# ZhengyiLuo/PHC

Measured on NVIDIA H100. Metric: env-steps/sec (fused obs+reward+PPO) at 4096 envs/GPU, higher is better.
Workload: dtype f32

## Files before the change

phc_b200/csrc/gemm_wgmma.cu:

```cuda
#include <cuda_runtime.h>
#include <stdint.h>
#include <stdlib.h>
#include <string.h>

#include "../../include/phc_b200.h"
#include "phc_common.cuh"

extern "C" void phc_set_error(const char* msg);
extern "C" int phc_check_cuda(cudaError_t e, const char* what);
extern "C" void phc_count_launches(int n);

namespace phc {
namespace wg {

constexpr int BM = 128, NUM_THREADS = 256, MAX_PROBLEMS = PHC_GEMM_GROUP_MAX;

template <int BN>
struct Cfg {
  static constexpr int BK = BN == 128 ? 32 : 16;
  static constexpr int A_TILE = BM * BK * 4;
  static constexpr int B_TILE = BN * BK * 4;
  static constexpr int STAGE = 2 * (A_TILE + B_TILE);
  static constexpr int SMEM = 2 * STAGE;
  static constexpr int SBO = BK * 32;
  static constexpr int A_PER = BM * BK / NUM_THREADS;
  static constexpr int B_PER = BN * BK / NUM_THREADS;
};

struct Prob {
  const float* A; const float* B; const float* A_lo; const float* B_lo;
  float* C; float* C_hi; float* C_lo;
  const float* bias;
  float* aux;
  long long lda, ldb, ldc, ldaux;
  int M, N, K;
  float alpha;
  int act, accumulate, a_k, b_k, k_splits;
  int tiles_m, tiles_n, kb_total, kb_per, tile_begin, tile_count;
  unsigned int* turn;
  int turn_first, turn_total;
};

struct Params {
  Prob p[MAX_PROBLEMS];
  int count, total_tiles;
  unsigned int* sched;
  int single_pass;
};

__device__ __forceinline__ void wgmma_tf32_n128(float (&d)[64], uint64_t da, uint64_t db) {
  asm volatile(
      "{\n\t.reg .pred p;\n\tsetp.ne.b32 p, 1, 0;\n\t"
      "wgmma.mma_async.sync.aligned.m64n128k8.f32.tf32.tf32 {%0, %1, %2, %3, %4, %5, %6, %7, %8, %9, %10, %11, %12, %13, %14, %15, %16, %17, %18, %19, %20, %21, %22, %23, %24, %25, %26, %27, %28, %29, %30, %31, %32, %33, %34, %35, %36, %37, %38, %39, %40, %41, %42, %43, %44, %45, %46, %47, %48, %49, %50, %51, %52, %53, %54, %55, %56, %57, %58, %59, %60, %61, %62, %63}, %64, %65, p, 1, 1;\n\t}"
      : "+f"(d[0]), "+f"(d[1]), "+f"(d[2]), "+f"(d[3]), "+f"(d[4]), "+f"(d[5]), "+f"(d[6]), "+f"(d[7]), "+f"(d[8]), "+f"(d[9]), "+f"(d[10]), "+f"(d[11]), "+f"(d[12]), "+f"(d[13]), "+f"(d[14]), "+f"(d[15]), "+f"(d[16]), "+f"(d[17]), "+f"(d[18]), "+f"(d[19]), "+f"(d[20]), "+f"(d[21]), "+f"(d[22]), "+f"(d[23]), "+f"(d[24]), "+f"(d[25]), "+f"(d[26]), "+f"(d[27]), "+f"(d[28]), "+f"(d[29]), "+f"(d[30]), "+f"(d[31]), "+f"(d[32]), "+f"(d[33]), "+f"(d[34]), "+f"(d[35]), "+f"(d[36]), "+f"(d[37]), "+f"(d[38]), "+f"(d[39]), "+f"(d[40]), "+f"(d[41]), "+f"(d[42]), "+f"(d[43]), "+f"(d[44]), "+f"(d[45]), "+f"(d[46]), "+f"(d[47]), "+f"(d[48]), "+f"(d[49]), "+f"(d[50]), "+f"(d[51]), "+f"(d[52]), "+f"(d[53]), "+f"(d[54]), "+f"(d[55]), "+f"(d[56]), "+f"(d[57]), "+f"(d[58]), "+f"(d[59]), "+f"(d[60]), "+f"(d[61]), "+f"(d[62]), "+f"(d[63])
      : "l"(da), "l"(db));
}
__device__ __forceinline__ void wgmma_tf32_n256(float (&d)[128], uint64_t da, uint64_t db) {
  asm volatile(
      "{\n\t.reg .pred p;\n\tsetp.ne.b32 p, 1, 0;\n\t"
      "wgmma.mma_async.sync.aligned.m64n256k8.f32.tf32.tf32 {%0, %1, %2, %3, %4, %5, %6, %7, %8, %9, %10, %11, %12, %13, %14, %15, %16, %17, %18, %19, %20, %21, %22, %23, %24, %25, %26, %27, %28, %29, %30, %31, %32, %33, %34, %35, %36, %37, %38, %39, %40, %41, %42, %43, %44, %45, %46, %47, %48, %49, %50, %51, %52, %53, %54, %55, %56, %57, %58, %59, %60, %61, %62, %63, %64, %65, %66, %67, %68, %69, %70, %71, %72, %73, %74, %75, %76, %77, %78, %79, %80, %81, %82, %83, %84, %85, %86, %87, %88, %89, %90, %91, %92, %93, %94, %95, %96, %97, %98, %99, %100, %101, %102, %103, %104, %105, %106, %107, %108, %109, %110, %111, %112, %113, %114, %115, %116, %117, %118, %119, %120, %121, %122, %123, %124, %125, %126, %127}, %128, %129, p, 1, 1;\n\t}"
      : "+f"(d[0]), "+f"(d[1]), "+f"(d[2]), "+f"(d[3]), "+f"(d[4]), "+f"(d[5]), "+f"(d[6]), "+f"(d[7]), "+f"(d[8]), "+f"(d[9]), "+f"(d[10]), "+f"(d[11]), "+f"(d[12]), "+f"(d[13]), "+f"(d[14]), "+f"(d[15]), "+f"(d[16]), "+f"(d[17]), "+f"(d[18]), "+f"(d[19]), "+f"(d[20]), "+f"(d[21]), "+f"(d[22]), "+f"(d[23]), "+f"(d[24]), "+f"(d[25]), "+f"(d[26]), "+f"(d[27]), "+f"(d[28]), "+f"(d[29]), "+f"(d[30]), "+f"(d[31]), "+f"(d[32]), "+f"(d[33]), "+f"(d[34]), "+f"(d[35]), "+f"(d[36]), "+f"(d[37]), "+f"(d[38]), "+f"(d[39]), "+f"(d[40]), "+f"(d[41]), "+f"(d[42]), "+f"(d[43]), "+f"(d[44]), "+f"(d[45]), "+f"(d[46]), "+f"(d[47]), "+f"(d[48]), "+f"(d[49]), "+f"(d[50]), "+f"(d[51]), "+f"(d[52]), "+f"(d[53]), "+f"(d[54]), "+f"(d[55]), "+f"(d[56]), "+f"(d[57]), "+f"(d[58]), "+f"(d[59]), "+f"(d[60]), "+f"(d[61]), "+f"(d[62]), "+f"(d[63]), "+f"(d[64]), "+f"(d[65]), "+f"(d[66]), "+f"(d[67]), "+f"(d[68]), "+f"(d[69]), "+f"(d[70]), "+f"(d[71]), "+f"(d[72]), "+f"(d[73]), "+f"(d[74]), "+f"(d[75]), "+f"(d[76]), "+f"(d[77]), "+f"(d[78]), "+f"(d[79]), "+f"(d[80]), "+f"(d[81]), "+f"(d[82]), "+f"(d[83]), "+f"(d[84]), "+f"(d[85]), "+f"(d[86]), "+f"(d[87]), "+f"(d[88]), "+f"(d[89]), "+f"(d[90]), "+f"(d[91]), "+f"(d[92]), "+f"(d[93]), "+f"(d[94]), "+f"(d[95]), "+f"(d[96]), "+f"(d[97]), "+f"(d[98]), "+f"(d[99]), "+f"(d[100]), "+f"(d[101]), "+f"(d[102]), "+f"(d[103]), "+f"(d[104]), "+f"(d[105]), "+f"(d[106]), "+f"(d[107]), "+f"(d[108]), "+f"(d[109]), "+f"(d[110]), "+f"(d[111]), "+f"(d[112]), "+f"(d[113]), "+f"(d[114]), "+f"(d[115]), "+f"(d[116]), "+f"(d[117]), "+f"(d[118]), "+f"(d[119]), "+f"(d[120]), "+f"(d[121]), "+f"(d[122]), "+f"(d[123]), "+f"(d[124]), "+f"(d[125]), "+f"(d[126]), "+f"(d[127])
      : "l"(da), "l"(db));
}

__device__ __forceinline__ void wgmma_fence() { asm volatile("wgmma.fence.sync.aligned;" ::: "memory"); }
__device__ __forceinline__ void wgmma_commit() { asm volatile("wgmma.commit_group.sync.aligned;" ::: "memory"); }
__device__ __forceinline__ void wgmma_wait_all() { asm volatile("wgmma.wait_group.sync.aligned 0;" ::: "memory"); }

__device__ __forceinline__ uint64_t smem_desc(uint32_t addr, uint32_t lbo, uint32_t sbo) {
  return (uint64_t)((addr & 0x3FFFF) >> 4) | ((uint64_t)(lbo >> 4) << 16) | ((uint64_t)(sbo >> 4) << 32);
}

template <int BN, typename Acc>
__device__ __forceinline__ void wgmma_tf32(Acc& d, uint64_t da, uint64_t db) {
  if constexpr (BN == 128) wgmma_tf32_n128(d, da, db); else wgmma_tf32_n256(d, da, db);
}

__device__ __forceinline__ float trunc_hi(float x) { return __uint_as_float(__float_as_uint(x) & 0xFFFFE000u); }
__device__ __forceinline__ float split_lo(float x) {
  const float d = x - trunc_hi(x);
  return __uint_as_float((__float_as_uint(d) + 0x1000u) & 0xFFFFE000u);
}
__device__ __forceinline__ void sts128(uint32_t addr, float a, float b, float c, float d) {
  asm volatile("st.shared.v4.f32 [%0], {%1, %2, %3, %4};" ::"r"(addr), "f"(a), "f"(b), "f"(c), "f"(d) : "memory");
}
__device__ __forceinline__ void sts32(uint32_t addr, float a) { asm volatile("st.shared.f32 [%0], %1;" ::"r"(addr), "f"(a) : "memory"); }

template <int R, int BK>
struct Map {
  static constexpr int KC = BK / 4;
  __device__ static void kmaj(int c, int& r, int& kc) { r = (c & 7) + 8 * (c / (8 * KC)); kc = (c >> 3) % KC; }
  __device__ static void mnmaj(int e, int& r, int& k, uint32_t& off) {
    const int rl = e & 7, kl = (e >> 3) & 3, e2 = e >> 5, rh = e2 % (R / 8), kh = e2 / (R / 8);
    r = rh * 8 + rl; k = kh * 4 + kl;
    off = (uint32_t)(rh * BK * 32 + kh * 128 + rl * 16 + kl * 4);
  }
};

template <int R, int BK, int PER>
__device__ __forceinline__ void load_op(float (&v)[PER], const float* __restrict__ g, long long ld, bool kmaj, int r0, int rows, int k0,
                                        int K, int tid) {
  using Mp = Map<R, BK>;
  if (kmaj) {
#pragma unroll
    for (int i = 0; i < PER / 4; ++i) {
      int r, kc;
      Mp::kmaj(tid + i * NUM_THREADS, r, kc);
      const int rr = r0 + r, kk = k0 + 4 * kc;
      const float* src = g + (long long)rr * ld + kk;
      if (rr < rows && kk + 3 < K) {
        const float4 t = *reinterpret_cast<const float4*>(src);
        v[4 * i] = t.x; v[4 * i + 1] = t.y; v[4 * i + 2] = t.z; v[4 * i + 3] = t.w;
      } else {
#pragma unroll
        for (int e = 0; e < 4; ++e) v[4 * i + e] = (rr < rows && kk + e < K) ? src[e] : 0.f;
      }
    }
  } else {
#pragma unroll
    for (int i = 0; i < PER; ++i) {
      int r, k;
      uint32_t off;
      Mp::mnmaj(tid + i * NUM_THREADS, r, k, off);
      const int rr = r0 + r, kk = k0 + k;
      v[i] = (rr < rows && kk < K) ? g[(long long)kk * ld + rr] : 0.f;
    }
  }
}

template <int R, int BK, int PER, int MODE>
__device__ __forceinline__ void store_op(const float (&v)[PER], const float (&w)[PER], uint32_t s_hi, uint32_t s_lo, bool kmaj, int tid) {
  using Mp = Map<R, BK>;
  auto hi = [](float x) { return MODE == 2 ? x : trunc_hi(x); };
  if (kmaj) {
#pragma unroll
    for (int i = 0; i < PER / 4; ++i) {
      const uint32_t off = (uint32_t)(tid + i * NUM_THREADS) * 16u;
      sts128(s_hi + off, hi(v[4 * i]), hi(v[4 * i + 1]), hi(v[4 * i + 2]), hi(v[4 * i + 3]));
      if (MODE == 0) sts128(s_lo + off, split_lo(v[4 * i]), split_lo(v[4 * i + 1]), split_lo(v[4 * i + 2]), split_lo(v[4 * i + 3]));
      if (MODE == 2) sts128(s_lo + off, w[4 * i], w[4 * i + 1], w[4 * i + 2], w[4 * i + 3]);
    }
  } else {
#pragma unroll
    for (int i = 0; i < PER; ++i) {
      int r, k;
      uint32_t off;
      Mp::mnmaj(tid + i * NUM_THREADS, r, k, off);
      sts32(s_hi + off, hi(v[i]));
      if (MODE == 0) sts32(s_lo + off, split_lo(v[i]));
      if (MODE == 2) sts32(s_lo + off, w[i]);
    }
  }
}

__device__ __forceinline__ void split_rna(float x, float& h, float& l) {
  uint32_t a, b;
  asm("cvt.rna.tf32.f32 %0, %1;" : "=r"(a) : "f"(x));
  const float res = x - __uint_as_float(a);
  asm("cvt.rna.tf32.f32 %0, %1;" : "=r"(b) : "f"(res));
  h = __uint_as_float(a); l = __uint_as_float(b);
}

template <int BN, bool PRESPLIT>
__global__ void __launch_bounds__(NUM_THREADS, 1) gemm_wgmma_kernel(const __grid_constant__ Params P) {
  using C = Cfg<BN>;
  constexpr int BK = C::BK;
  extern __shared__ __align__(128) uint8_t smem[];
  __shared__ int s_tile;
  const int tid = threadIdx.x, lane = tid & 31, wgi = tid >> 7, wq = (tid >> 5) & 3;
  const uint32_t sbase = (uint32_t)__cvta_generic_to_shared(smem);
  const bool dyn = P.sched != nullptr;
  const bool single = !PRESPLIT && P.single_pass != 0;

  for (int it = 0;; ++it) {
    int t;
    if (dyn) {
      if (tid == 0) s_tile = (int)atomicAdd(P.sched, 1u);
      __syncthreads();
      t = s_tile;
      __syncthreads();
    } else {
      t = blockIdx.x + it * gridDim.x;
    }
    if (t >= P.total_tiles) break;
    int gi = 0;
#pragma unroll 1
    while (gi + 1 < P.count && t >= P.p[gi].tile_begin + P.p[gi].tile_count) ++gi;
    const Prob& q = P.p[gi];
    const int tl = t - q.tile_begin;
    const int ni = tl % q.tiles_n, rr = tl / q.tiles_n, mi = rr % q.tiles_m, z = rr / q.tiles_m;
    const int m0 = mi * BM, n0 = ni * BN;
    const int kb_begin = z * q.kb_per;
    const int nkb = max(0, min(q.kb_total, kb_begin + q.kb_per) - kb_begin);
    if (nkb == 0) continue;
    const bool ak = q.a_k != 0, bk = q.b_k != 0;

    float acc[BN / 2];
#pragma unroll
    for (int j = 0; j < BN / 2; ++j) acc[j] = 0.f;
    float va[C::A_PER], vb[C::B_PER], wa[PRESPLIT ? C::A_PER : 1], wb[PRESPLIT ? C::B_PER : 1];
    constexpr int MODE = PRESPLIT ? 2 : 0;
    auto load = [&](int kb) {
      const int k0 = kb * BK;
      load_op<BM, BK>(va, q.A, q.lda, ak, m0, q.M, k0, q.K, tid);
      load_op<BN, BK>(vb, q.B, q.ldb, bk, n0, q.N, k0, q.K, tid);
      if constexpr (PRESPLIT) {
        load_op<BM, BK>(wa, q.A_lo, q.lda, ak, m0, q.M, k0, q.K, tid);
        load_op<BN, BK>(wb, q.B_lo, q.ldb, bk, n0, q.N, k0, q.K, tid);
      }
    };
    auto store = [&](int buf) {
      const uint32_t s = sbase + (uint32_t)(buf * C::STAGE);
      if (single) {
        store_op<BM, BK, C::A_PER, 1>(va, va, s, 0, ak, tid);
        store_op<BN, BK, C::B_PER, 1>(vb, vb, s + 2 * C::A_TILE, 0, bk, tid);
      } else if constexpr (PRESPLIT) {
        store_op<BM, BK, C::A_PER, 2>(va, wa, s, s + C::A_TILE, ak, tid);
        store_op<BN, BK, C::B_PER, 2>(vb, wb, s + 2 * C::A_TILE, s + 2 * C::A_TILE + C::B_TILE, bk, tid);
      } else {
        store_op<BM, BK, C::A_PER, MODE>(va, va, s, s + C::A_TILE, ak, tid);
        store_op<BN, BK, C::B_PER, MODE>(vb, vb, s + 2 * C::A_TILE, s + 2 * C::A_TILE + C::B_TILE, bk, tid);
      }
      fence_async_smem();
    };

    load(kb_begin);
    store(0);
    __syncthreads();
#pragma unroll 1
    for (int i = 0; i < nkb; ++i) {
      const uint32_t s = sbase + (uint32_t)((i & 1) * C::STAGE);
      const uint32_t a_hi = s + (uint32_t)(wgi * 8 * C::SBO), a_lo = a_hi + C::A_TILE;
      const uint32_t b_hi = s + 2 * C::A_TILE, b_lo = b_hi + C::B_TILE;
      wgmma_fence();
#pragma unroll
      for (int kk = 0; kk < BK / 8; ++kk) {
        const uint32_t o = (uint32_t)kk * 256u;
        const uint64_t dAh = smem_desc(a_hi + o, 128, C::SBO), dBh = smem_desc(b_hi + o, 128, C::SBO);
        if (!single) {
          wgmma_tf32<BN>(acc, smem_desc(a_lo + o, 128, C::SBO), dBh);
          wgmma_tf32<BN>(acc, dAh, smem_desc(b_lo + o, 128, C::SBO));
        }
        wgmma_tf32<BN>(acc, dAh, dBh);
      }
      wgmma_commit();
      if (i + 1 < nkb) {
        load(kb_begin + i + 1);
        store((i + 1) & 1);
      }
      wgmma_wait_all();
      __syncthreads();
    }

    const bool ordered = q.turn != nullptr;
    volatile unsigned int* turn = ordered ? q.turn + mi * q.tiles_n + ni : nullptr;
    if (ordered) {
      if (tid == 0) {
        while (*turn != (unsigned)(q.turn_first + z)) __nanosleep(64);
        __threadfence();
      }
      __syncthreads();
    }
    const int act = q.act;
    const float* bias = (q.bias && z == 0) ? q.bias : nullptr;
#pragma unroll
    for (int h = 0; h < 2; ++h) {
      const int m = m0 + wgi * 64 + wq * 16 + (lane >> 2) + 8 * h;
      const bool row_ok = m < q.M;
      float* crow = q.C + (long long)m * q.ldc;
      float* arow = (q.aux && act < PHC_ACT_RELU_BITS && row_ok) ? q.aux + (long long)m * q.ldaux : nullptr;
      uint32_t* brow = (q.aux && act >= PHC_ACT_RELU_BITS && row_ok) ? reinterpret_cast<uint32_t*>(q.aux) + (long long)m * q.ldaux : nullptr;
#pragma unroll
      for (int qc = 0; qc < BN / 32; ++qc) {
        const int nb = n0 + 32 * qc;
        if (nb >= q.N) break;
        const uint32_t mbits = (act == PHC_ACT_MASK_BITS && brow) ? brow[nb >> 5] : 0u;
        uint32_t bits = 0;
#pragma unroll
        for (int jj = 0; jj < 4; ++jj) {
          const int j = 4 * qc + jj;
          const int nl = 8 * jj + 2 * (lane & 3);
          float v[2];
#pragma unroll
          for (int c = 0; c < 2; ++c) {
            const int n = nb + nl + c;
            float x = q.alpha * acc[4 * j + 2 * h + c];
            if (bias && n < q.N) x += bias[n];
            if (act == PHC_ACT_RELU || act == PHC_ACT_RELU_BITS) x = fmaxf(x, 0.f);
            if (act == PHC_ACT_RELU_BITS) bits |= (x > 0.f ? 1u : 0u) << (nl + c);
            else if (act == PHC_ACT_MASK_BITS) x = ((mbits >> (nl + c)) & 1u) ? x : 0.f;
            else if (arow && n < q.N) {
              if (act == PHC_ACT_SILU) { arow[n] = x; x = silu_f(x); }
              else if (act == PHC_ACT_SILU_BWD) x *= silu_grad_f(arow[n]);
              else x = arow[n] > 0.f ? x : 0.f;
// ... 1 lines not shown
              x = silu_f(x);
            }
            v[c] = x;
          }
          if (!row_ok) continue;
          const int n = nb + nl;
          if (ordered) {
            if (n < q.N) crow[n] = __ldcg(crow + n) + v[0];
            if (n + 1 < q.N) crow[n + 1] = __ldcg(crow + n + 1) + v[1];
          } else if (q.accumulate) {
            if (n < q.N) atomicAdd(crow + n, v[0]);
            if (n + 1 < q.N) atomicAdd(crow + n + 1, v[1]);
          } else if (n + 1 < q.N) {
            *reinterpret_cast<float2*>(crow + n) = make_float2(v[0], v[1]);
          } else if (n < q.N) {
            crow[n] = v[0];
          }
          if (PRESPLIT && q.C_hi) {
            float h0, l0, h1, l1;
            split_rna(v[0], h0, l0); split_rna(v[1], h1, l1);
            if (n < q.N) { q.C_hi[(long long)m * q.ldc + n] = h0; q.C_lo[(long long)m * q.ldc + n] = l0; }
            if (n + 1 < q.N) { q.C_hi[(long long)m * q.ldc + n + 1] = h1; q.C_lo[(long long)m * q.ldc + n + 1] = l1; }
          }
        }
        if (act == PHC_ACT_RELU_BITS) {
          bits |= __shfl_xor_sync(0xffffffffu, bits, 1);
          bits |= __shfl_xor_sync(0xffffffffu, bits, 2);
          if (brow && (lane & 3) == 0) brow[nb >> 5] = bits;
        }
      }
    }
    if (ordered) {
      __threadfence();
      __syncthreads();
      if (tid == 0) *turn = (q.turn_first + z + 1 == q.turn_total) ? 0u : (unsigned)(q.turn_first + z + 1);
    }
  }
  if (dyn && tid == 0 && atomicInc(P.sched + 1, gridDim.x - 1) == gridDim.x - 1) { __threadfence(); P.sched[0] = 0u; }
}

__global__ void split_lo_kernel(const float* __restrict__ x, float* __restrict__ lo, int64_t n) {
  const int64_t stride = (int64_t)gridDim.x * blockDim.x;
  for (int64_t i = (int64_t)blockIdx.x * blockDim.x + threadIdx.x; i < n; i += stride) lo[i] = split_lo(x[i]);
}

__global__ void split_tf32_kernel(const float* __restrict__ x, int64_t ldx, int64_t rows, int cols, float* __restrict__ hi,
                                  float* __restrict__ lo, int64_t ldo) {
  const int64_t total = rows * cols;
  for (int64_t i = (int64_t)blockIdx.x * blockDim.x + threadIdx.x; i < total; i += (int64_t)gridDim.x * blockDim.x) {
    const int64_t r = i / cols;
    const int c = (int)(i - r * cols);
    split_rna(x[r * ldx + c], hi[r * ldo + c], lo[r * ldo + c]);
  }
}

static int g_single_pass = 0;
static int g_tile = 0;
static int g_sched = -1;
constexpr int SCHED_SLOTS = 64;
__device__ unsigned int g_sched_counters[SCHED_SLOTS][2];
constexpr int TURN_SLOTS = 16, TURN_TILES = 8192;
__device__ unsigned int g_turns[TURN_SLOTS][TURN_TILES];

static int num_sms() {
  static int n = 0;
  if (!n) { int dev = 0; cudaGetDevice(&dev); cudaDeviceGetAttribute(&n, cudaDevAttrMultiProcessorCount, dev); if (n <= 0) n = 132; }
  return n;
}

static int add_problem(Params& P, int n, int tiles, int bn, const float* A, const float* A_lo, long long lda, int a_k, const float* B,
                       const float* B_lo, long long ldb, int b_k, float* Cm, float* C_hi, float* C_lo, long long ldc, int M, int N, int K,
                       float alpha, const float* bias, int act, float* aux, long long ldaux, int accumulate, int k_splits) {
  const int bk = bn == 128 ? Cfg<128>::BK : Cfg<256>::BK;
  Prob& q = P.p[n];
  q.A = A; q.A_lo = A_lo; q.B = B; q.B_lo = B_lo; q.C = Cm; q.C_hi = C_hi; q.C_lo = C_lo; q.bias = bias; q.aux = aux;
  q.lda = lda; q.ldb = ldb; q.ldc = ldc; q.ldaux = ldaux; q.M = M; q.N = N; q.K = K; q.alpha = alpha; q.act = act;
  q.accumulate = accumulate ? 1 : 0; q.a_k = a_k ? 1 : 0; q.b_k = b_k ? 1 : 0;
  int ks = k_splits < 1 ? 1 : k_splits;
  q.tiles_m = (M + BM - 1) / BM;
  q.tiles_n = (N + bn - 1) / bn;
  q.kb_total = (K + bk - 1) / bk;
  if (ks > q.kb_total) ks = q.kb_total;
  q.kb_per = (q.kb_total + ks - 1) / ks;
  ks = (q.kb_total + q.kb_per - 1) / q.kb_per;
  q.k_splits = ks;
  q.turn = nullptr;
  q.tile_begin = tiles;
  q.tile_count = q.tiles_m * q.tiles_n * ks;
  return q.tile_count;
}

template <int BN, bool PRESPLIT>
static int launch(Params& P, bool dynamic_sched, cudaStream_t stream) {
  int owner[MAX_PROBLEMS];
  bool ordered = false;
  int turn_tiles = 0;
  for (int i = 0; i < P.count; ++i) {
    Prob& q = P.p[i];
    owner[i] = -1;
    for (int j = 0; j < i && q.accumulate; ++j) {
// ... 20 lines not shown
      void* p = nullptr;
      cudaError_t es = cudaGetSymbolAddress(&p, g_turns);
      if (es != cudaSuccess) return phc_check_cuda(es, "cudaGetSymbolAddress(g_turns)");
      tbase = static_cast<unsigned int*>(p);
    }
    unsigned int* t = tbase + (size_t)(turn_no++ % TURN_SLOTS) * TURN_TILES;
    for (int i = 0; i < P.count; ++i) {
      Prob& q = P.p[i];
      if (owner[i] >= 0) {
        Prob& o = P.p[owner[i]];
        q.turn = o.turn;
        q.turn_first = o.turn_total;
        o.turn_total += q.k_splits;
      } else if (q.k_splits > 1 || has_members[i]) {
        q.turn = t; t += q.tiles_m * q.tiles_n;
      }
    }
    for (int i = 0; i < P.count; ++i)
      if (owner[i] >= 0) P.p[i].turn_total = P.p[owner[i]].turn_total;
    dynamic_sched = true;
  }
  P.sched = nullptr;
  if (dynamic_sched) {
    static unsigned int* base = nullptr;
    static unsigned int launch_no = 0;
    if (!base) {
      void* p = nullptr;
      cudaError_t es = cudaGetSymbolAddress(&p, g_sched_counters);
      if (es != cudaSuccess) return phc_check_cuda(es, "cudaGetSymbolAddress(g_sched_counters)");
      base = static_cast<unsigned int*>(p);
    }
    P.sched = base + 2 * (launch_no++ % SCHED_SLOTS);
  }
  static bool smem_set = false;
  if (!smem_set) {
    cudaError_t e = cudaFuncSetAttribute(gemm_wgmma_kernel<BN, PRESPLIT>, cudaFuncAttributeMaxDynamicSharedMemorySize, Cfg<BN>::SMEM);
    if (e != cudaSuccess) return phc_check_cuda(e, "cudaFuncSetAttribute(gemm_wgmma)");
    smem_set = true;
  }
  const int sms = num_sms();
  const unsigned grid = (unsigned)(P.total_tiles < sms ? P.total_tiles : sms);
  gemm_wgmma_kernel<BN, PRESPLIT><<<grid, NUM_THREADS, Cfg<BN>::SMEM, stream>>>(P);
  phc_count_launches(1);
  return phc_check_cuda(cudaGetLastError(), "gemm_wgmma_kernel launch");
}

}
}

static int validate_group(const PhcGemmDesc* d, int32_t count) {
  using namespace phc::wg;
  if (!d || count < 1 || count > MAX_PROBLEMS) { phc_set_error("phc_gemm_group: 1 <= count <= PHC_GEMM_GROUP_MAX problems"); return PHC_ERR_INVALID_ARG; }
  for (int i = 0; i < count; ++i) {
    const PhcGemmDesc& g = d[i];
    if (!g.A || !g.B || !g.C || g.M < 0 || g.N < 0 || g.K < 1) { phc_set_error("phc_gemm_group: bad problem (NULL operand or negative size)"); return PHC_ERR_INVALID_ARG; }
    if (g.M == 0 || g.N == 0) continue;
    if ((g.lda & 3) || (g.ldb & 3) || (g.ldc & 3)) { phc_set_error("phc_gemm_group: leading dimensions must be multiples of 4 floats (16-byte operand loads)"); return PHC_ERR_INVALID_ARG; }
    for (const void* p : {(const void*)g.A, (const void*)g.B, (const void*)g.C})
      if (reinterpret_cast<uintptr_t>(p) & 15) { phc_set_error("phc_gemm_group: A, B, C must be 16-byte aligned"); return PHC_ERR_INVALID_ARG; }
    const int ks = g.k_splits < 1 ? 1 : g.k_splits;
    if (g.act < 0 || g.act > PHC_ACT_MASK_BITS || ((g.act == PHC_ACT_SILU_BWD || g.act == PHC_ACT_MASK_BITS) && !g.aux)) { phc_set_error("phc_gemm_group: bad activation code"); return PHC_ERR_INVALID_ARG; }
    if (g.act >= PHC_ACT_RELU_BITS && g.aux && ((reinterpret_cast<uintptr_t>(g.aux) & 3) || g.ldaux < (g.N + 31) / 32)) { phc_set_error("phc_gemm_group: bit-mask aux needs ldaux >= ceil(N / 32) words"); return PHC_ERR_INVALID_ARG; }
    if (ks > 1 && (!g.accumulate || g.act || g.aux)) { phc_set_error("phc_gemm_group: split-K needs accumulate=1 and a linear epilogue"); return PHC_ERR_INVALID_ARG; }
    if (g.B_lo && (reinterpret_cast<uintptr_t>(g.B_lo) & 15)) { phc_set_error("phc_gemm_group: B_lo must be 16-byte aligned"); return PHC_ERR_INVALID_ARG; }
  }
  auto span = [](const PhcGemmDesc& g, uintptr_t& lo, uintptr_t& hi) {
    lo = reinterpret_cast<uintptr_t>(g.C);
    hi = lo + (uintptr_t)(((int64_t)g.M - 1) * g.ldc + g.N) * sizeof(float);
  };
  for (int i = 0; i < count; ++i) {
    const PhcGemmDesc& a = d[i];
    if (a.M == 0 || a.N == 0) continue;
    uintptr_t a0, a1;
    span(a, a0, a1);
    for (int j = 0; j < i; ++j) {
      const PhcGemmDesc& b = d[j];
      if (b.M == 0 || b.N == 0) continue;
      uintptr_t b0, b1;
      span(b, b0, b1);
      if (a0 >= b1 || b0 >= a1) continue;
      if (a.accumulate && b.accumulate && a.C == b.C && a.M == b.M && a.N == b.N && a.ldc == b.ldc) continue;
      phc_set_error("phc_gemm_group: two problems write overlapping C ranges (only accumulating problems on the same C with the same M, N, ldc may)");
      return PHC_ERR_INVALID_ARG;
    }
  }
  return PHC_OK;
}

extern "C" int phc_gemm_group(const PhcGemmDesc* d, int32_t count, void* stream) {
  using namespace phc::wg;
// ... 5 lines not shown
  memset(&P, 0, sizeof(P));
  int tiles = 0, n = 0;
  for (int i = 0; i < count; ++i) {
    const PhcGemmDesc& g = d[i];
    if (g.M == 0 || g.N == 0) continue;
    tiles += add_problem(P, n, tiles, bn, g.A, nullptr, g.lda, g.a_kmajor, g.B, nullptr, g.ldb, g.b_kmajor, g.C, nullptr, nullptr, g.ldc,
                         g.M, g.N, g.K, g.alpha, g.bias, g.act, g.aux, g.ldaux, g.accumulate, g.k_splits);
    ++n;
  }
  if (n == 0) return PHC_OK;
  P.count = n; P.total_tiles = tiles; P.single_pass = g_single_pass;
  cudaStream_t st = static_cast<cudaStream_t>(stream);
  return bn == 256 ? launch<256, false>(P, g_sched == 1, st) : launch<128, false>(P, g_sched == 1, st);
}

extern "C" int phc_gemm_tc5s(const float* A, int64_t lda, int32_t a_kmajor, const float* B, int64_t ldb, int32_t b_kmajor, float* C,
                             int64_t ldc, int32_t M, int32_t N, int32_t K, float alpha, const float* bias, int32_t act, float* aux,
                             int64_t ldaux, int32_t accumulate, int32_t k_splits, void* stream) {
  PhcGemmDesc d;
  d.A = A; d.lda = lda; d.a_kmajor = a_kmajor; d.B = B; d.ldb = ldb; d.b_kmajor = b_kmajor; d.C = C; d.ldc = ldc;
  d.M = M; d.N = N; d.K = K; d.alpha = alpha; d.bias = bias; d.act = act; d.aux = aux; d.ldaux = ldaux;
  d.accumulate = accumulate; d.k_splits = k_splits; d.B_lo = nullptr;
  return phc_gemm_group(&d, 1, stream);
}

extern "C" int phc_gemm_tc5(const float* A_hi, const float* A_lo, int64_t lda, int32_t a_kmajor, const float* B_hi,
                            const float* B_lo, int64_t ldb, int32_t b_kmajor, float* C, float* C_hi, float* C_lo, int64_t ldc,
                            int32_t M, int32_t N, int32_t K, float alpha, const float* bias, int32_t relu, float* mask,
                            int64_t ldmask, int32_t accumulate, int32_t k_splits, void* stream) {
  using namespace phc::wg;
  if (!A_hi || !A_lo || !B_hi || !B_lo || !C || M < 0 || N < 0 || K < 1) { phc_set_error("phc_gemm_tc5: bad arguments"); return PHC_ERR_INVALID_ARG; }
  if (M == 0 || N == 0) return PHC_OK;
  if ((lda & 3) || (ldb & 3) || (ldc & 1)) { phc_set_error("phc_gemm_tc5: lda, ldb must be multiples of 4 floats, ldc of 2"); return PHC_ERR_INVALID_ARG; }
  for (const void* p : {(const void*)A_hi, (const void*)A_lo, (const void*)B_hi, (const void*)B_lo})
    if (reinterpret_cast<uintptr_t>(p) & 15) { phc_set_error("phc_gemm_tc5: operands must be 16-byte aligned"); return PHC_ERR_INVALID_ARG; }
  if (reinterpret_cast<uintptr_t>(C) & 7) { phc_set_error("phc_gemm_tc5: C must be 8-byte aligned"); return PHC_ERR_INVALID_ARG; }
  if (k_splits < 1) k_splits = 1;
  if (relu < 0 || relu > PHC_ACT_SILU_BWD || (relu == PHC_ACT_SILU_BWD && !mask)) { phc_set_error("phc_gemm_tc5: bad activation code"); return PHC_ERR_INVALID_ARG; }
  if (k_splits > 1 && (!accumulate || relu || mask)) { phc_set_error("phc_gemm_tc5: split-K needs accumulate=1 and a linear epilogue"); return PHC_ERR_INVALID_ARG; }
  if ((C_hi == nullptr) != (C_lo == nullptr) || (C_hi && accumulate)) { phc_set_error("phc_gemm_tc5: C_hi/C_lo come as a pair and not with accumulate"); return PHC_ERR_INVALID_ARG; }
  static Params P;
  memset(&P, 0, sizeof(P));
  P.total_tiles = add_problem(P, 0, 0, 128, A_hi, A_lo, lda, a_kmajor, B_hi, B_lo, ldb, b_kmajor, C, C_hi, C_lo, ldc, M, N, K, alpha, bias,
                              relu, mask, ldmask, accumulate, k_splits);
  P.count = 1;
  return launch<128, true>(P, false, static_cast<cudaStream_t>(stream));
}

extern "C" int phc_split_tf32(const float* x, int64_t ldx, int64_t rows, int32_t cols, float* hi, float* lo, int64_t ldo,
                              void* stream) {
  if (!x || !hi || !lo || rows < 0 || cols < 1 || ldx < cols || ldo < cols) { phc_set_error("phc_split_tf32: bad arguments"); return PHC_ERR_INVALID_ARG; }
  if (rows == 0) return PHC_OK;
  int64_t g = (rows * cols + 255) / 256; if (g > 132 * 8) g = 132 * 8;
  phc::wg::split_tf32_kernel<<<(unsigned)g, 256, 0, static_cast<cudaStream_t>(stream)>>>(x, ldx, rows, cols, hi, lo, ldo);
  phc_count_launches(1);
  return phc_check_cuda(cudaGetLastError(), "split_tf32_kernel");
}

extern "C" int phc_split_lo(const float* x, float* lo, int64_t n, void* stream) {
  if (n < 0 || (n > 0 && (!x || !lo))) { phc_set_error("phc_split_lo: NULL buffer"); return PHC_ERR_INVALID_ARG; }
  if (n == 0) return PHC_OK;
  const int threads = 256;
  int64_t blocks = (n + threads - 1) / threads;
  if (blocks > 132 * 8) blocks = 132 * 8;
  phc::wg::split_lo_kernel<<<(unsigned)blocks, threads, 0, static_cast<cudaStream_t>(stream)>>>(x, lo, n);
  phc_count_launches(1);
// ... 26 lines not shown
```

Measured before the change: 192,600.

## Feed wgmma GEMM via TMA producer warp with mbarrier ring and swizzled split

Replaces the register-staged global loads in the TF32 wgmma GEMM with a dedicated producer warpgroup that issues TMA bulk tensor loads into a multi-stage raw-tile ring guarded by mbarriers. Consumer warpgroups copy from the raw stage into a swizzled hi/lo split buffer before running wgmma, and registers are rebalanced with setmaxnreg. Tensor maps are encoded on the host and kept in a hash cache. The aim is to overlap global memory latency with MMA work and cut bank conflicts, at the cost of more shared memory, per-launch host map encoding, an extra smem-to-smem split pass, and new lda/ldb validity checks.

Result: faster. 225,900, median of 6 (+17.3%).

```diff
diff --git a/phc_b200/csrc/gemm_ring.cuh b/phc_b200/csrc/gemm_ring.cuh
--- /dev/null
+++ b/phc_b200/csrc/gemm_ring.cuh
@@ -0,0 +1,24 @@
+#pragma once
+
+#if defined(__CUDACC__)
+#define PHC_RING_HD __host__ __device__ __forceinline__
+#else
+#define PHC_RING_HD inline
+#endif
+
+namespace phc {
+namespace ring {
+
+template <int S>
+struct Pos {
+  int stage = 0;
+  unsigned phase = 0;
+  PHC_RING_HD unsigned full_parity() const { return phase; }
+  PHC_RING_HD unsigned empty_parity() const { return phase ^ 1u; }
+  PHC_RING_HD void advance() {
+    if (++stage == S) { stage = 0; phase ^= 1u; }
+  }
+};
+
+}
+}
diff --git a/phc_b200/csrc/gemm_wgmma.cu b/phc_b200/csrc/gemm_wgmma.cu
--- a/phc_b200/csrc/gemm_wgmma.cu
+++ b/phc_b200/csrc/gemm_wgmma.cu
@@ -1,9 +1,12 @@
+#include <cuda.h>
+#include <cudaTypedefs.h>
 #include <cuda_runtime.h>
 #include <stdint.h>
 #include <stdlib.h>
 #include <string.h>
 
 #include "../../include/phc_b200.h"
+#include "gemm_ring.cuh"
 #include "phc_common.cuh"
 
 extern "C" void phc_set_error(const char* msg);
@@ -14,6 +17,7 @@
 namespace wg {
 
 constexpr int BM = 128, NUM_THREADS = 256, MAX_PROBLEMS = PHC_GEMM_GROUP_MAX;
+constexpr int CTA_THREADS = NUM_THREADS + 128;
 
 template <int BN>
 struct Cfg {
@@ -21,10 +25,17 @@
   static constexpr int A_TILE = BM * BK * 4;
   static constexpr int B_TILE = BN * BK * 4;
   static constexpr int STAGE = 2 * (A_TILE + B_TILE);
-  static constexpr int SMEM = 2 * STAGE;
-  static constexpr int SBO = BK * 32;
-  static constexpr int A_PER = BM * BK / NUM_THREADS;
-  static constexpr int B_PER = BN * BK / NUM_THREADS;
+};
+
+template <int BN, bool PRESPLIT>
+struct Smem {
+  using C = Cfg<BN>;
+  static constexpr int RAW = (PRESPLIT ? 2 : 1) * (C::A_TILE + C::B_TILE);
+  static constexpr int STAGES = PRESPLIT ? 1 : BN == 128 ? 3 : 4;
+  static constexpr int SPLIT = STAGES * RAW;
+  static constexpr int BARS = SPLIT + 2 * C::STAGE;
+  static constexpr int TILE_IDS = BARS + 16 * STAGES;
+  static constexpr int BYTES = TILE_IDS + 4 * STAGES;
 };
 
 struct Prob {
@@ -42,6 +53,8 @@
 };
 
 struct Params {
+  CUtensorMap map[MAX_PROBLEMS][2];
+  CUtensorMap map_lo[2];
   Prob p[MAX_PROBLEMS];
   int count, total_tiles;
   unsigned int* sched;
@@ -85,74 +98,6 @@
   asm volatile("st.shared.v4.f32 [%0], {%1, %2, %3, %4};" ::"r"(addr), "f"(a), "f"(b), "f"(c), "f"(d) : "memory");
 }
 __device__ __forceinline__ void sts32(uint32_t addr, float a) { asm volatile("st.shared.f32 [%0], %1;" ::"r"(addr), "f"(a) : "memory"); }
-
-template <int R, int BK>
-struct Map {
-  static constexpr int KC = BK / 4;
-  __device__ static void kmaj(int c, int& r, int& kc) { r = (c & 7) + 8 * (c / (8 * KC)); kc = (c >> 3) % KC; }
-  __device__ static void mnmaj(int e, int& r, int& k, uint32_t& off) {
-    const int rl = e & 7, kl = (e >> 3) & 3, e2 = e >> 5, rh = e2 % (R / 8), kh = e2 / (R / 8);
-    r = rh * 8 + rl; k = kh * 4 + kl;
-    off = (uint32_t)(rh * BK * 32 + kh * 128 + rl * 16 + kl * 4);
-  }
-};
-
-template <int R, int BK, int PER>
-__device__ __forceinline__ void load_op(float (&v)[PER], const float* __restrict__ g, long long ld, bool kmaj, int r0, int rows, int k0,
-                                        int K, int tid) {
-  using Mp = Map<R, BK>;
-  if (kmaj) {
-#pragma unroll
-    for (int i = 0; i < PER / 4; ++i) {
-      int r, kc;
-      Mp::kmaj(tid + i * NUM_THREADS, r, kc);
-      const int rr = r0 + r, kk = k0 + 4 * kc;
-      const float* src = g + (long long)rr * ld + kk;
-      if (rr < rows && kk + 3 < K) {
-        const float4 t = *reinterpret_cast<const float4*>(src);
-        v[4 * i] = t.x; v[4 * i + 1] = t.y; v[4 * i + 2] = t.z; v[4 * i + 3] = t.w;
-      } else {
-#pragma unroll
-        for (int e = 0; e < 4; ++e) v[4 * i + e] = (rr < rows && kk + e < K) ? src[e] : 0.f;
-      }
-    }
-  } else {
-#pragma unroll
-    for (int i = 0; i < PER; ++i) {
-      int r, k;
-      uint32_t off;
-      Mp::mnmaj(tid + i * NUM_THREADS, r, k, off);
-      const int rr = r0 + r, kk = k0 + k;
-      v[i] = (rr < rows && kk < K) ? g[(long long)kk * ld + rr] : 0.f;
-    }
-  }
-}
-
-template <int R, int BK, int PER, int MODE>
-__device__ __forceinline__ void store_op(const float (&v)[PER], const float (&w)[PER], uint32_t s_hi, uint32_t s_lo, bool kmaj, int tid) {
-  using Mp = Map<R, BK>;
-  auto hi = [](float x) { return MODE == 2 ? x : trunc_hi(x); };
-  if (kmaj) {
-#pragma unroll
-    for (int i = 0; i < PER / 4; ++i) {
-      const uint32_t off = (uint32_t)(tid + i * NUM_THREADS) * 16u;
-      sts128(s_hi + off, hi(v[4 * i]), hi(v[4 * i + 1]), hi(v[4 * i + 2]), hi(v[4 * i + 3]));
-      if (MODE == 0) sts128(s_lo + off, split_lo(v[4 * i]), split_lo(v[4 * i + 1]), split_lo(v[4 * i + 2]), split_lo(v[4 * i + 3]));
-      if (MODE == 2) sts128(s_lo + off, w[4 * i], w[4 * i + 1], w[4 * i + 2], w[4 * i + 3]);
-    }
-  } else {
-#pragma unroll
-    for (int i = 0; i < PER; ++i) {
-      int r, k;
-      uint32_t off;
-      Mp::mnmaj(tid + i * NUM_THREADS, r, k, off);
-      sts32(s_hi + off, hi(v[i]));
-      if (MODE == 0) sts32(s_lo + off, split_lo(v[i]));
-      if (MODE == 2) sts32(s_lo + off, w[i]);
-    }
-  }
-}
-
 __device__ __forceinline__ void split_rna(float x, float& h, float& l) {
   uint32_t a, b;
   asm("cvt.rna.tf32.f32 %0, %1;" : "=r"(a) : "f"(x));
@@ -161,95 +106,243 @@
   h = __uint_as_float(a); l = __uint_as_float(b);
 }
 
+__device__ __forceinline__ float4 lds128(uint32_t addr) {
+  float4 v;
+  asm volatile("ld.shared.v4.f32 {%0, %1, %2, %3}, [%4];" : "=f"(v.x), "=f"(v.y), "=f"(v.z), "=f"(v.w) : "r"(addr) : "memory");
+  return v;
+}
+__device__ __forceinline__ float lds32(uint32_t addr) {
+  float v;
+  asm volatile("ld.shared.f32 %0, [%1];" : "=f"(v) : "r"(addr) : "memory");
+  return v;
+}
+
+__device__ __forceinline__ void mbar_init(uint32_t bar, uint32_t count) {
+  asm volatile("mbarrier.init.shared::cta.b64 [%0], %1;" ::"r"(bar), "r"(count) : "memory");
+}
+__device__ __forceinline__ void mbar_arrive(uint32_t bar) {
+  asm volatile("mbarrier.arrive.shared::cta.b64 _, [%0];" ::"r"(bar) : "memory");
+}
+__device__ __forceinline__ void mbar_arrive_expect_tx(uint32_t bar, uint32_t bytes) {
+  asm volatile("mbarrier.arrive.expect_tx.shared::cta.b64 _, [%0], %1;" ::"r"(bar), "r"(bytes) : "memory");
+}
+__device__ __forceinline__ void mbar_wait(uint32_t bar, uint32_t parity) {
+  asm volatile(
+      "{\n\t.reg .pred p;\n\t"
+      "WAIT:\n\t"
+      "mbarrier.try_wait.parity.shared::cta.b64 p, [%0], %1;\n\t"
+      "@!p bra WAIT;\n\t}" ::"r"(bar), "r"(parity) : "memory");
+}
+__device__ __forceinline__ void tma_load_2d(uint32_t dst, const CUtensorMap* map, uint32_t bar, int c0, int c1) {
+  asm volatile("cp.async.bulk.tensor.2d.shared::cluster.global.mbarrier::complete_tx::bytes [%0], [%1, {%2, %3}], [%4];"
+               ::"r"(dst), "l"(reinterpret_cast<uint64_t>(map)), "r"(c0), "r"(c1), "r"(bar) : "memory");
+}
+__device__ __forceinline__ void consumer_sync() { asm volatile("bar.sync 1, 256;" ::: "memory"); }
+
+template <int BK>
+struct Sw {
+  static constexpr int ROW = BK * 4, SBO = 8 * ROW;
+  static constexpr uint64_t TYPE = BK == 32 ? 1 : 2;
+  __device__ static uint32_t off(int r, int c) { return (uint32_t)(r * ROW + ((c ^ (BK == 32 ? (r & 7) : ((r >> 1) & 3))) * 16)); }
+  __device__ static uint64_t desc(uint32_t addr) { return smem_desc(addr, 16, SBO) | (TYPE << 62); }
+};
+
+template <int R, int BK, int MODE>
+__device__ __forceinline__ void split_kmaj(uint32_t raw, uint32_t raw_lo, uint32_t s_hi, uint32_t s_lo, int tid) {
+  constexpr int KC = BK / 4, PER = R * KC / NUM_THREADS;
+  float4 v[PER], w[MODE == 2 ? PER : 1];
+#pragma unroll
+  for (int i = 0; i < PER; ++i) {
+    const int c = tid + i * NUM_THREADS, r = c / KC, kc = c % KC;
+    v[i] = lds128(raw + (uint32_t)(r * BK * 4 + kc * 16));
+    if constexpr (MODE == 2) w[i] = lds128(raw_lo + (uint32_t)(r * BK * 4 + kc * 16));
+  }
+#pragma unroll
+  for (int i = 0; i < PER; ++i) {
+    const int c = tid + i * NUM_THREADS, r = c / KC, kc = c % KC;
+    const uint32_t dst = Sw<BK>::off(r, kc);
+    if constexpr (MODE == 2) {
+      sts128(s_hi + dst, v[i].x, v[i].y, v[i].z, v[i].w);
+      sts128(s_lo + dst, w[i].x, w[i].y, w[i].z, w[i].w);
+    } else {
+      sts128(s_hi + dst, trunc_hi(v[i].x), trunc_hi(v[i].y), trunc_hi(v[i].z), trunc_hi(v[i].w));
+      if (MODE == 0) sts128(s_lo + dst, split_lo(v[i].x), split_lo(v[i].y), split_lo(v[i].z), split_lo(v[i].w));
+    }
+  }
+}
+
+template <int R, int BK, int MODE>
+__device__ __forceinline__ void split_mnmaj(uint32_t raw, uint32_t raw_lo, uint32_t s_hi, uint32_t s_lo, int tid) {
+  constexpr int RW = R / 32, PER = R * BK / NUM_THREADS, G = 8;
+  auto where = [&](int i, uint32_t& src, uint32_t& dst) {
+    const int e = tid + i * NUM_THREADS, lane = e & 31, x = (e >> 5) & 3, w = e >> 7;
+    const int r = (w % RW) * 32 + lane, kh = w / RW, k = kh * 4 + (((lane >> 3) + x) & 3);
+    src = (uint32_t)((k * R + r) * 4);
+    dst = Sw<BK>::off(r, kh) + (uint32_t)((k & 3) * 4);
+  };
+#pragma unroll 1
+  for (int i0 = 0; i0 < PER; i0 += G) {
+    float v[G], w[MODE == 2 ? G : 1];
+#pragma unroll
+    for (int i = 0; i < G; ++i) {
+      uint32_t src, dst;
+      where(i0 + i, src, dst);
+      v[i] = lds32(raw + src);
+      if constexpr (MODE == 2) w[i] = lds32(raw_lo + src);
+    }
+#pragma unroll
+    for (int i = 0; i < G; ++i) {
+      uint32_t src, dst;
+      where(i0 + i, src, dst);
+      if constexpr (MODE == 2) {
+        sts32(s_hi + dst, v[i]);
+        sts32(s_lo + dst, w[i]);
+      } else {
+        sts32(s_hi + dst, trunc_hi(v[i]));
+        if (MODE == 0) sts32(s_lo + dst, split_lo(v[i]));
+      }
+    }
+  }
+}
+
+template <int R, int BK, int MODE>
+__device__ __forceinline__ void split_op(bool kmaj, uint32_t raw, uint32_t raw_lo, uint32_t s_hi, uint32_t s_lo, int tid) {
+  if (kmaj) split_kmaj<R, BK, MODE>(raw, raw_lo, s_hi, s_lo, tid);
+  else split_mnmaj<R, BK, MODE>(raw, raw_lo, s_hi, s_lo, tid);
+}
+
+struct Tile {
+  int gi, mi, ni, z, kb_begin, nkb;
+};
+__device__ __forceinline__ Tile decode_tile(const Params& P, int t) {
+  Tile d;
+  d.gi = 0;
+#pragma unroll 1
+  while (d.gi + 1 < P.count && t >= P.p[d.gi].tile_begin + P.p[d.gi].tile_count) ++d.gi;
+  const Prob& q = P.p[d.gi];
+  const int tl = t - q.tile_begin;
+  const int rr = tl / q.tiles_n;
+  d.ni = tl % q.tiles_n; d.mi = rr % q.tiles_m; d.z = rr / q.tiles_m;
+  d.kb_begin = d.z * q.kb_per;
+  d.nkb = max(0, min(q.kb_total, d.kb_begin + q.kb_per) - d.kb_begin);
+  return d;
+}
+
+__device__ __forceinline__ void load_box(uint32_t dst, const CUtensorMap* map, bool kmaj, int r0, int k0, uint32_t bar) {
+  if (kmaj) tma_load_2d(dst, map, bar, k0, r0);
+  else tma_load_2d(dst, map, bar, r0, k0);
+}
+
 template <int BN, bool PRESPLIT>
-__global__ void __launch_bounds__(NUM_THREADS, 1) gemm_wgmma_kernel(const __grid_constant__ Params P) {
+__global__ void __launch_bounds__(CTA_THREADS, 1) gemm_wgmma_kernel(const __grid_constant__ Params P) {
   using C = Cfg<BN>;
-  constexpr int BK = C::BK;
-  extern __shared__ __align__(128) uint8_t smem[];
-  __shared__ int s_tile;
-  const int tid = threadIdx.x, lane = tid & 31, wgi = tid >> 7, wq = (tid >> 5) & 3;
+  using L = Smem<BN, PRESPLIT>;
+  constexpr int BK = C::BK, S = L::STAGES;
+  extern __shared__ __align__(1024) uint8_t smem[];
+  const int tid = threadIdx.x;
   const uint32_t sbase = (uint32_t)__cvta_generic_to_shared(smem);
+  const uint32_t full0 = sbase + L::BARS, empty0 = full0 + 8 * S;
+  volatile int* tile_id = reinterpret_cast<volatile int*>(smem + L::TILE_IDS);
   const bool dyn = P.sched != nullptr;
+
+  if (tid == 0) {
+    for (int s = 0; s < S; ++s) { mbar_init(full0 + 8 * s, 1); mbar_init(empty0 + 8 * s, NUM_THREADS / 32); }
+    asm volatile("fence.mbarrier_init.release.cluster;" ::: "memory");
+  }
+  __syncthreads();
+
+  if (tid >= NUM_THREADS) {
+    asm volatile("setmaxnreg.dec.sync.aligned.u32 40;" ::: "memory");
+    if (tid != NUM_THREADS) return;
+    ring::Pos<S> rp;
+#pragma unroll 1
+    for (int it = 0;; ++it) {
+      const int t = dyn ? (int)atomicAdd(P.sched, 1u) : (int)(blockIdx.x + it * gridDim.x);
+      if (t >= P.total_tiles) break;
+      const Tile d = decode_tile(P, t);
+      const Prob& q = P.p[d.gi];
+#pragma unroll 1
+      for (int i = 0; i < d.nkb; ++i) {
+        mbar_wait(empty0 + 8 * rp.stage, rp.empty_parity());
+        tile_id[rp.stage] = t;
+        const uint32_t bar = full0 + 8 * rp.stage, st = sbase + (uint32_t)(rp.stage * L::RAW);
+        const int k0 = (d.kb_begin + i) * BK;
+        mbar_arrive_expect_tx(bar, L::RAW);
+        load_box(st, &P.map[d.gi][0], q.a_k != 0, d.mi * BM, k0, bar);
+        load_box(st + C::A_TILE, &P.map[d.gi][1], q.b_k != 0, d.ni * BN, k0, bar);
+        if constexpr (PRESPLIT) {
+          load_box(st + C::A_TILE + C::B_TILE, &P.map_lo[0], q.a_k != 0, d.mi * BM, k0, bar);
+          load_box(st + 2 * C::A_TILE + C::B_TILE, &P.map_lo[1], q.b_k != 0, d.ni * BN, k0, bar);
+        }
+        rp.advance();
+      }
+    }
+    mbar_wait(empty0 + 8 * rp.stage, rp.empty_parity());
+    tile_id[rp.stage] = -1;
+    mbar_arrive(full0 + 8 * rp.stage);
+    if (dyn && atomicInc(P.sched + 1, gridDim.x - 1) == gridDim.x - 1) { __threadfence(); P.sched[0] = 0u; }
+    return;
+  }
+
+  asm volatile("setmaxnreg.inc.sync.aligned.u32 232;" ::: "memory");
+  const int lane = tid & 31, wgi = tid >> 7, wq = (tid >> 5) & 3;
   const bool single = !PRESPLIT && P.single_pass != 0;
-
-  for (int it = 0;; ++it) {
-    int t;
-    if (dyn) {
-      if (tid == 0) s_tile = (int)atomicAdd(P.sched, 1u);
-      __syncthreads();
-      t = s_tile;
-      __syncthreads();
-    } else {
-      t = blockIdx.x + it * gridDim.x;
-    }
-    if (t >= P.total_tiles) break;
-    int gi = 0;
+  const uint32_t split0 = sbase + L::SPLIT;
+  ring::Pos<S> rc;
 #pragma unroll 1
-    while (gi + 1 < P.count && t >= P.p[gi].tile_begin + P.p[gi].tile_count) ++gi;
-    const Prob& q = P.p[gi];
-    const int tl = t - q.tile_begin;
-    const int ni = tl % q.tiles_n, rr = tl / q.tiles_n, mi = rr % q.tiles_m, z = rr / q.tiles_m;
+  for (;;) {
+    mbar_wait(full0 + 8 * rc.stage, rc.full_parity());
+    const int t = tile_id[rc.stage];
+    if (t < 0) break;
+    const Tile d = decode_tile(P, t);
+    const Prob& q = P.p[d.gi];
+    const int mi = d.mi, ni = d.ni, z = d.z, nkb = d.nkb;
     const int m0 = mi * BM, n0 = ni * BN;
-    const int kb_begin = z * q.kb_per;
-    const int nkb = max(0, min(q.kb_total, kb_begin + q.kb_per) - kb_begin);
-    if (nkb == 0) continue;
     const bool ak = q.a_k != 0, bk = q.b_k != 0;
 
     float acc[BN / 2];
 #pragma unroll
     for (int j = 0; j < BN / 2; ++j) acc[j] = 0.f;
-    float va[C::A_PER], vb[C::B_PER], wa[PRESPLIT ? C::A_PER : 1], wb[PRESPLIT ? C::B_PER : 1];
-    constexpr int MODE = PRESPLIT ? 2 : 0;
-    auto load = [&](int kb) {
-      const int k0 = kb * BK;
-      load_op<BM, BK>(va, q.A, q.lda, ak, m0, q.M, k0, q.K, tid);
-      load_op<BN, BK>(vb, q.B, q.ldb, bk, n0, q.N, k0, q.K, tid);
-      if constexpr (PRESPLIT) {
-        load_op<BM, BK>(wa, q.A_lo, q.lda, ak, m0, q.M, k0, q.K, tid);
-        load_op<BN, BK>(wb, q.B_lo, q.ldb, bk, n0, q.N, k0, q.K, tid);
+    auto split = [&](int buf) {
+      mbar_wait(full0 + 8 * rc.stage, rc.full_parity());
+      const uint32_t raw = sbase + (uint32_t)(rc.stage * L::RAW), s = split0 + (uint32_t)(buf * C::STAGE);
+      const uint32_t raw_lo = raw + C::A_TILE + C::B_TILE;
+      if (single) {
+        split_op<BM, BK, 1>(ak, raw, 0, s, 0, tid);
+        split_op<BN, BK, 1>(bk, raw + C::A_TILE, 0, s + 2 * C::A_TILE, 0, tid);
+      } else {
+        constexpr int MODE = PRESPLIT ? 2 : 0;
+        split_op<BM, BK, MODE>(ak, raw, raw_lo, s, s + C::A_TILE, tid);
+        split_op<BN, BK, MODE>(bk, raw + C::A_TILE, raw_lo + C::A_TILE, s + 2 * C::A_TILE, s + 2 * C::A_TILE + C::B_TILE, tid);
       }
-    };
-    auto store = [&](int buf) {
-      const uint32_t s = sbase + (uint32_t)(buf * C::STAGE);
-      if (single) {
-        store_op<BM, BK, C::A_PER, 1>(va, va, s, 0, ak, tid);
-        store_op<BN, BK, C::B_PER, 1>(vb, vb, s + 2 * C::A_TILE, 0, bk, tid);
-      } else if constexpr (PRESPLIT) {
-        store_op<BM, BK, C::A_PER, 2>(va, wa, s, s + C::A_TILE, ak, tid);
-        store_op<BN, BK, C::B_PER, 2>(vb, wb, s + 2 * C::A_TILE, s + 2 * C::A_TILE + C::B_TILE, bk, tid);
-      } else {
-        store_op<BM, BK, C::A_PER, MODE>(va, va, s, s + C::A_TILE, ak, tid);
-        store_op<BN, BK, C::B_PER, MODE>(vb, vb, s + 2 * C::A_TILE, s + 2 * C::A_TILE + C::B_TILE, bk, tid);
-      }
+      __syncwarp();
+      if (lane == 0) mbar_arrive(empty0 + 8 * rc.stage);
+      rc.advance();
       fence_async_smem();
     };
 
-    load(kb_begin);
-    store(0);
-    __syncthreads();
+    split(0);
+    consumer_sync();
 #pragma unroll 1
     for (int i = 0; i < nkb; ++i) {
-      const uint32_t s = sbase + (uint32_t)((i & 1) * C::STAGE);
-      const uint32_t a_hi = s + (uint32_t)(wgi * 8 * C::SBO), a_lo = a_hi + C::A_TILE;
+      const uint32_t s = split0 + (uint32_t)((i & 1) * C::STAGE);
+      const uint32_t a_hi = s + (uint32_t)(wgi * 64 * Sw<BK>::ROW), a_lo = a_hi + C::A_TILE;
       const uint32_t b_hi = s + 2 * C::A_TILE, b_lo = b_hi + C::B_TILE;
       wgmma_fence();
 #pragma unroll
       for (int kk = 0; kk < BK / 8; ++kk) {
-        const uint32_t o = (uint32_t)kk * 256u;
-        const uint64_t dAh = smem_desc(a_hi + o, 128, C::SBO), dBh = smem_desc(b_hi + o, 128, C::SBO);
+        const uint32_t o = (uint32_t)kk * 32u;
+        const uint64_t dAh = Sw<BK>::desc(a_hi + o), dBh = Sw<BK>::desc(b_hi + o);
         if (!single) {
-          wgmma_tf32<BN>(acc, smem_desc(a_lo + o, 128, C::SBO), dBh);
-          wgmma_tf32<BN>(acc, dAh, smem_desc(b_lo + o, 128, C::SBO));
+          wgmma_tf32<BN>(acc, Sw<BK>::desc(a_lo + o), dBh);
+          wgmma_tf32<BN>(acc, dAh, Sw<BK>::desc(b_lo + o));
         }
         wgmma_tf32<BN>(acc, dAh, dBh);
       }
       wgmma_commit();
-      if (i + 1 < nkb) {
-        load(kb_begin + i + 1);
-        store((i + 1) & 1);
-      }
+      if (i + 1 < nkb) split((i + 1) & 1);
       wgmma_wait_all();
-      __syncthreads();
+      consumer_sync();
     }
 
     const bool ordered = q.turn != nullptr;
@@ -259,7 +352,7 @@
         while (*turn != (unsigned)(q.turn_first + z)) __nanosleep(64);
         __threadfence();
       }
-      __syncthreads();
+      consumer_sync();
     }
     const int act = q.act;
     const float* bias = (q.bias && z == 0) ? q.bias : nullptr;
@@ -327,11 +420,10 @@
     }
     if (ordered) {
       __threadfence();
-      __syncthreads();
+      consumer_sync();
       if (tid == 0) *turn = (q.turn_first + z + 1 == q.turn_total) ? 0u : (unsigned)(q.turn_first + z + 1);
     }
   }
-  if (dyn && tid == 0 && atomicInc(P.sched + 1, gridDim.x - 1) == gridDim.x - 1) { __threadfence(); P.sched[0] = 0u; }
 }
 
 __global__ void split_lo_kernel(const float* __restrict__ x, float* __restrict__ lo, int64_t n) {
@@ -361,6 +453,58 @@
   static int n = 0;
   if (!n) { int dev = 0; cudaGetDevice(&dev); cudaDeviceGetAttribute(&n, cudaDevAttrMultiProcessorCount, dev); if (n <= 0) n = 132; }
   return n;
+}
+
+struct MapKey {
+  const float* ptr;
+  long long rows, K, ld;
+  int kmaj, box_rows, bk;
+  bool operator==(const MapKey& o) const {
+    return ptr == o.ptr && rows == o.rows && K == o.K && ld == o.ld && kmaj == o.kmaj && box_rows == o.box_rows && bk == o.bk;
+  }
+};
+constexpr int MAP_CACHE = 1024, MAP_PROBE = 8;
+static MapKey g_map_key[MAP_CACHE];
+static CUtensorMap g_map_val[MAP_CACHE];
+static bool g_map_set[MAP_CACHE];
+
+static unsigned map_hash(const MapKey& k) {
+  unsigned long long h = reinterpret_cast<uintptr_t>(k.ptr) >> 4;
+  for (long long v : {k.rows, k.K, k.ld, (long long)k.kmaj, (long long)k.box_rows, (long long)k.bk}) h = (h ^ (unsigned long long)v) * 0x100000001b3ull;
+  return (unsigned)(h ^ (h >> 29));
+}
+
+static int tensor_map(CUtensorMap* out, const float* ptr, bool kmaj, long long rows, long long K, long long ld, int box_rows, int bk) {
+  const MapKey key{ptr, rows, K, ld, kmaj ? 1 : 0, box_rows, bk};
+  const unsigned h = map_hash(key);
+  int slot = -1;
+  for (int i = 0; i < MAP_PROBE; ++i) {
+    const int j = (int)((h + i) % MAP_CACHE);
+    if (g_map_set[j] && g_map_key[j] == key) { *out = g_map_val[j]; return PHC_OK; }
+    if (!g_map_set[j] && slot < 0) slot = j;
+  }
+  if (slot < 0) slot = (int)(h % MAP_CACHE);
+  static PFN_cuTensorMapEncodeTiled encode = nullptr;
+  if (!encode) {
+    void* fn = nullptr;
+    cudaDriverEntryPointQueryResult qr;
+    const cudaError_t e = cudaGetDriverEntryPoint("cuTensorMapEncodeTiled", &fn, cudaEnableDefault, &qr);
+    if (e != cudaSuccess) return phc_check_cuda(e, "cudaGetDriverEntryPoint(cuTensorMapEncodeTiled)");
+    if (qr != cudaDriverEntryPointSuccess || !fn) { phc_set_error("gemm: the driver has no cuTensorMapEncodeTiled"); return PHC_ERR_CUDA; }
+    encode = reinterpret_cast<PFN_cuTensorMapEncodeTiled>(fn);
+  }
+  const cuuint64_t dim[2] = {(cuuint64_t)(kmaj ? K : rows), (cuuint64_t)(kmaj ? rows : K)};
+  const cuuint64_t stride[1] = {(cuuint64_t)ld * sizeof(float)};
+  const cuuint32_t box[2] = {(cuuint32_t)(kmaj ? bk : box_rows), (cuuint32_t)(kmaj ? box_rows : bk)};
+  const cuuint32_t estride[2] = {1, 1};
+  const CUresult r = encode(out, CU_TENSOR_MAP_DATA_TYPE_FLOAT32, 2, const_cast<float*>(ptr), dim, stride, box, estride,
+                            CU_TENSOR_MAP_INTERLEAVE_NONE, CU_TENSOR_MAP_SWIZZLE_NONE, CU_TENSOR_MAP_L2_PROMOTION_L2_128B,
+                            CU_TENSOR_MAP_FLOAT_OOB_FILL_NONE);
+  if (r != CUDA_SUCCESS) { phc_set_error("gemm: cuTensorMapEncodeTiled refused an operand (leading dimension smaller than its row?)"); return PHC_ERR_INVALID_ARG; }
+  g_map_set[slot] = true;
+  g_map_key[slot] = key;
+  g_map_val[slot] = *out;
+  return PHC_OK;
 }
 
 static int add_problem(Params& P, int n, int tiles, int bn, const float* A, const float* A_lo, long long lda, int a_k, const float* B,
@@ -447,15 +591,25 @@
     }
     P.sched = base + 2 * (launch_no++ % SCHED_SLOTS);
   }
+  constexpr int BK = Cfg<BN>::BK;
+  for (int i = 0; i < P.count; ++i) {
+    const Prob& q = P.p[i];
+    int rc = tensor_map(&P.map[i][0], q.A, q.a_k != 0, q.M, q.K, q.lda, BM, BK);
+    if (rc == PHC_OK) rc = tensor_map(&P.map[i][1], q.B, q.b_k != 0, q.N, q.K, q.ldb, BN, BK);
+    if (rc == PHC_OK && PRESPLIT) rc = tensor_map(&P.map_lo[0], q.A_lo, q.a_k != 0, q.M, q.K, q.lda, BM, BK);
+    if (rc == PHC_OK && PRESPLIT) rc = tensor_map(&P.map_lo[1], q.B_lo, q.b_k != 0, q.N, q.K, q.ldb, BN, BK);
+    if (rc != PHC_OK) return rc;
+  }
+  constexpr int SMEM = Smem<BN, PRESPLIT>::BYTES;
   static bool smem_set = false;
   if (!smem_set) {
-    cudaError_t e = cudaFuncSetAttribute(gemm_wgmma_kernel<BN, PRESPLIT>, cudaFuncAttributeMaxDynamicSharedMemorySize, Cfg<BN>::SMEM);
+    cudaError_t e = cudaFuncSetAttribute(gemm_wgmma_kernel<BN, PRESPLIT>, cudaFuncAttributeMaxDynamicSharedMemorySize, SMEM);
     if (e != cudaSuccess) return phc_check_cuda(e, "cudaFuncSetAttribute(gemm_wgmma)");
     smem_set = true;
   }
   const int sms = num_sms();
   const unsigned grid = (unsigned)(P.total_tiles < sms ? P.total_tiles : sms);
-  gemm_wgmma_kernel<BN, PRESPLIT><<<grid, NUM_THREADS, Cfg<BN>::SMEM, stream>>>(P);
+  gemm_wgmma_kernel<BN, PRESPLIT><<<grid, CTA_THREADS, SMEM, stream>>>(P);
   phc_count_launches(1);
   return phc_check_cuda(cudaGetLastError(), "gemm_wgmma_kernel launch");
 }
@@ -471,6 +625,7 @@
     if (!g.A || !g.B || !g.C || g.M < 0 || g.N < 0 || g.K < 1) { phc_set_error("phc_gemm_group: bad problem (NULL operand or negative size)"); return PHC_ERR_INVALID_ARG; }
     if (g.M == 0 || g.N == 0) continue;
     if ((g.lda & 3) || (g.ldb & 3) || (g.ldc & 3)) { phc_set_error("phc_gemm_group: leading dimensions must be multiples of 4 floats (16-byte operand loads)"); return PHC_ERR_INVALID_ARG; }
+    if (g.lda < (g.a_kmajor ? g.K : g.M) || g.ldb < (g.b_kmajor ? g.K : g.N)) { phc_set_error("phc_gemm_group: lda / ldb must cover a row of the operand (>= K when k-contiguous, else >= M / N)"); return PHC_ERR_INVALID_ARG; }
     for (const void* p : {(const void*)g.A, (const void*)g.B, (const void*)g.C})
       if (reinterpret_cast<uintptr_t>(p) & 15) { phc_set_error("phc_gemm_group: A, B, C must be 16-byte aligned"); return PHC_ERR_INVALID_ARG; }
     const int ks = g.k_splits < 1 ? 1 : g.k_splits;
@@ -542,6 +697,7 @@
   if (!A_hi || !A_lo || !B_hi || !B_lo || !C || M < 0 || N < 0 || K < 1) { phc_set_error("phc_gemm_tc5: bad arguments"); return PHC_ERR_INVALID_ARG; }
   if (M == 0 || N == 0) return PHC_OK;
   if ((lda & 3) || (ldb & 3) || (ldc & 1)) { phc_set_error("phc_gemm_tc5: lda, ldb must be multiples of 4 floats, ldc of 2"); return PHC_ERR_INVALID_ARG; }
+  if (lda < (a_kmajor ? K : M) || ldb < (b_kmajor ? K : N)) { phc_set_error("phc_gemm_tc5: lda / ldb must cover a row of the operand (>= K when k-contiguous, else >= M / N)"); return PHC_ERR_INVALID_ARG; }
   for (const void* p : {(const void*)A_hi, (const void*)A_lo, (const void*)B_hi, (const void*)B_lo})
     if (reinterpret_cast<uintptr_t>(p) & 15) { phc_set_error("phc_gemm_tc5: operands must be 16-byte aligned"); return PHC_ERR_INVALID_ARG; }
   if (reinterpret_cast<uintptr_t>(C) & 7) { phc_set_error("phc_gemm_tc5: C must be 8-byte aligned"); return PHC_ERR_INVALID_ARG; }
```
